# snudm-starlab/VMLMF

Hardware: AMD Instinct MI355X
Metric: RNN timesteps/sec (fwd+bwd) at B=64 T=128 hid=180 r=16; 1/2/4/8 GPU (higher is better)
Workload: dtype f32; 1 GPU; BASELINE configs[1]: UCI-HAR shape, Net(MyLSTM[MyVMLMFCell]) 1 layer, B=64/GPU T=128 I=9 H=180 w_rank=16 u_rank=16, CE loss, fwd+bwd; parameters packed inside every step, as a training loop sees it (with kept parameter images: ms_per_step_kept_images); global_batch=64, batch_per_gpu=64, seq_len=128, parallelism=dp1, scaling=weak, launch=hipgraph, parameter_images=packed inside every step (what a training loop sees), criterion=vmlmf_amd.Net.loss (cross-entropy riding on the forward launch, C ABI vmlmf_ce)

## Files before the change

### vmlmf_amd/csrc/vmlmf_launch.h

```cpp
#pragma once
#include <hip/hip_runtime.h>
#include "vmlmf_device.h"
#include "vmlmf_dropout.h"

#define VG_REC_BOUNDS (MAXT + 128)

enum EnvRule { ENV_SET, ENV_ON, ENV_INT, ENV_POS };
int vmlmf_env_switch(const char* name, EnvRule rule, int dflt);

struct HeadFwd {
  const float *W, *bias;
  float* logits;
  int C, pad;
};
struct HeadBwd {
  const float *W, *dl;
  const float* hlast;
  float *dW, *db;
  long long ldh;
  int C, pad;
};

struct FwdArgs {
  const float *gx, *VE, *UR, *EH, *h0, *c0;
// ... 11 lines not shown
  unsigned long long* ticket;
};
struct XwArgs {
  const float *x, *UXP, *WXD, *BBT;
  HeadFwd hd;
  CeFwd ce;
  const float *BH, *DX;
  int direct, pad;
};
struct AtbArgs {
  const float *dpre, *x, *y, *h0, *qx, *dqx, *Qs, *dQs;
  float* P;
  int pad0, pad;
};
constexpr int WR_PROG_STRIDE = 32;
constexpr unsigned VMLMF_ST_WRIDE = 1, VMLMF_ST_CLUSTER = 2, VMLMF_ST_WF_FWD = 3, VMLMF_ST_WF_BWD = 4, VMLMF_ST_P2P = 5;
__device__ __forceinline__ void vg_raise(unsigned* status, unsigned code) {
  if (status != nullptr) __hip_atomic_store(status, code, __ATOMIC_RELAXED, __HIP_MEMORY_SCOPE_SYSTEM);
}
struct WRide {
  AtbArgs a;
  float* dux;
  const float* vx;
  unsigned* prog;
  int K, S, ntg, tasks;
  int lag;
  int direct;
  unsigned spin;
  unsigned* status;
};
// ... 290 lines not shown
```

### vmlmf_amd/csrc/vmlmf_rec3.inc

```
#include "vmlmf_rec_fwd.inc"
#include "vmlmf_rec_bwd.inc"

constexpr int R3_MAXS = 3;


__device__ __forceinline__ float r3_total(float4 p) { return (p.x + p.y) + (p.z + p.w); }

__device__ __forceinline__ float fmac_ror_x16_4(float src, const float* w) {
  float a0 = 0.f, a1 = 0.f, a2 = 0.f, a3 = 0.f;
  asm("v_fmac_f32 %0, %4, %5\n\t" VG_DPP1(1, 4, 6, 1) VG_DPP1(2, 4, 7, 2) VG_DPP1(3, 4, 8, 3) VG_DPP1(0, 4, 9, 4) VG_DPP1(1, 4, 10, 5)
      VG_DPP1(2, 4, 11, 6) VG_DPP1(3, 4, 12, 7) VG_DPP1(0, 4, 13, 8) VG_DPP1(1, 4, 14, 9) VG_DPP1(2, 4, 15, 10) VG_DPP1(3, 4, 16, 11)
      VG_DPP1(0, 4, 17, 12) VG_DPP1(1, 4, 18, 13) VG_DPP1(2, 4, 19, 14) VG_DPP1(3, 4, 20, 15)
      : "+v"(a0), "+v"(a1), "+v"(a2), "+v"(a3)
      : "v"(src), "v"(w[0]), "v"(w[1]), "v"(w[2]), "v"(w[3]), "v"(w[4]), "v"(w[5]), "v"(w[6]), "v"(w[7]), "v"(w[8]), "v"(w[9]),
        "v"(w[10]), "v"(w[11]), "v"(w[12]), "v"(w[13]), "v"(w[14]), "v"(w[15]));
  return (a0 + a1) + (a2 + a3);
}

__host__ __device__ inline size_t rec3_fwd_lds_floats(int NT, int T, int IM) { return 128 + (size_t)12 * NT + (size_t)(T + 32) * IM + 8; }

template <int KH, int IM>
__global__ void __launch_bounds__(256) rec3_fwd_kernel(VGeo g, FwdArgs a, XwArgs xwargs) {
  static_assert(KH == 8 || KH == 16, "one 16-rank pass");
  static_assert(IM % 4 == 0 && IM >= 4 && IM <= 16, "narrow inputs");
// ... 225 lines not shown
  }
  hipLaunchKernelGGL(kern, dim3(g.nwg), dim3(g.NT + 64), lds, s, g, a, xw);
  return (int)hipGetLastError();
}
template <int KH>
static int rec3_fwd_launch_kh(const VGeo& g, const FwdArgs& a, const XwArgs& xw, hipStream_t s) {
  switch ((g.I + 3) / 4) {
    case 1: return rec3_fwd_launch_one<KH, 4>(g, a, xw, s);
    case 2: return rec3_fwd_launch_one<KH, 8>(g, a, xw, s);
    case 3: return rec3_fwd_launch_one<KH, 12>(g, a, xw, s);
    case 4: return rec3_fwd_launch_one<KH, 16>(g, a, xw, s);
  }
  return -3;
}

__host__ __device__ inline size_t rec3_bwd_lds_floats(int NT) {
  return 128 + (size_t)BWD_NB * NT * 6 + (size_t)2 * NT * 4 + 256 + 4 + (size_t)DR_SCR_FLOATS * NT;
}

#define VG_ADD1(acc, src, k) "v_add_f32_dpp %" #acc ", %" #src ", %" #acc " row_ror:" #k " row_mask:0xf bank_mask:0xf\n\t"
__device__ __forceinline__ float add_ror_x16(const float (&z)[16]) {
  float a0 = z[0], a1 = 0.f, a2 = 0.f;
  asm("s_nop 1\n\t" VG_ADD1(1, 3, 1) VG_ADD1(2, 4, 2) VG_ADD1(0, 5, 3) VG_ADD1(1, 6, 4) VG_ADD1(2, 7, 5) VG_ADD1(0, 8, 6) VG_ADD1(1, 9, 7)
      VG_ADD1(2, 10, 8) VG_ADD1(0, 11, 9) VG_ADD1(1, 12, 10) VG_ADD1(2, 13, 11) VG_ADD1(0, 14, 12) VG_ADD1(1, 15, 13) VG_ADD1(2, 16, 14)
      VG_ADD1(0, 17, 15)
      : "+v"(a0), "+v"(a1), "+v"(a2)
      : "v"(z[1]), "v"(z[2]), "v"(z[3]), "v"(z[4]), "v"(z[5]), "v"(z[6]), "v"(z[7]), "v"(z[8]), "v"(z[9]), "v"(z[10]), "v"(z[11]),
        "v"(z[12]), "v"(z[13]), "v"(z[14]), "v"(z[15]));
  return (a0 + a1) + a2;
}

template <int KH, int RIDE = 0>
__global__ void __launch_bounds__(320) rec3_bwd_kernel(VGeo g, BwdArgs a) {
  static_assert(KH == 8 || KH == 16, "one 16-rank pass");
  if constexpr (RIDE > 0) {
    if ((int)blockIdx.x >= g.nwg) {
      wride_worker<RIDE>(g, a.wr);
      return;
    }
  }
  const int tid = threadIdx.x, lane = tid & 63, wave = tid >> 6;
  const int NT = g.NT, NW = g.NW, H = g.H, B = g.B, T = g.T;
  const bool has_dy = a.dy != nullptr;
  const size_t sstride = (size_t)g.Bp * NT;
  const int row = blockIdx.x;

  extern __shared__ float4 smem4[];
  float* part = reinterpret_cast<float*>(smem4);
  float* tg = part + 128;
  float* tcp = tg + BWD_NB * NT * 4;
  float* tdy = tcp + BWD_NB * NT;
  float* outs = tdy + BWD_NB * NT;
  float* spare = outs + 2 * NT * 4;
  float* drscr = spare + 256 + 4;
  if (tid < 128) part[tid] = 0.f;

  if (tid >= NT) {
    constexpr int MAXS = R3_MAXS;
    constexpr int NDMA = 3 * MAXS;
    constexpr int DEPTH = 2;
    constexpr int DIST = DEPTH + 2;
    static_assert(DIST < BWD_NB && 2 * NDMA <= 63, "tape ring");
    if (wave == NW) {
      auto issue = [&](int ttarget) {
        const int tc = ttarget > 0 ? ttarget : 0;
        const int ring = ((ttarget % BWD_NB) + BWD_NB) % BWD_NB;
#pragma unroll
        for (int i = 0; i < MAXS; ++i) {
          const bool real = i < NW;
          const int slot = lane + 64 * (real ? i : 0);
          const size_t e = (size_t)tc * sstride + (size_t)row * NT + slot;
          int n;
          if (!vg_slot_unit(g, slot, n)) n = 0;
          const size_t lo = (size_t)ring * NT + 64 * (real ? i : 0);
          dma16(a.gates + e * 4, real ? tg + lo * 4 : spare);
          dma4(a.cs + e, real ? tcp + lo : spare);
          dma4(has_dy ? a.dy + ((size_t)tc * g.syT + (size_t)row * g.syB + n) : a.cs + e, real ? tdy + lo : spare);
        }
      };
      for (int s0 = 0; s0 < DIST; ++s0) issue(T - 1 - s0);
      wait_vm_barrier<(DIST - 2) * NDMA>();
      for (int t = T - 1; t >= 0; --t) {
        issue(t - DIST);
        wait_vm_barrier<DEPTH * NDMA>();
      }
      return;
    }
    const bool qv = lane < KH;
    const unsigned qdst = (unsigned)(row * KH + (lane < KH ? lane : 0)) * 4u;
    constexpr bool SAFE_ST = false;
    auto drain = [&](int ts) {
      const float* src = outs + (size_t)(ts & 1) * NT * 4;
      float* dt = a.dpre + (size_t)ts * sstride * 4;
      float4 d4[MAXS];
#pragma unroll
      for (int i = 0; i < MAXS; ++i) d4[i] = ld4(src + ((size_t)lane + 64 * (i < NW ? i : 0)) * 4);
      const float4 pq = ld4(part + (ts & 1) * 64 + (lane & 15) * 4);
#pragma unroll
      for (int i = 0; i < MAXS; ++i)
        if (i < NW) {
          if constexpr (RIDE > 0) st4_sv_sys<SAFE_ST>(dt, 16u * (unsigned)(row * NT + lane + 64 * i), d4[i]);
          else st4_sv(dt, 16u * (unsigned)(row * NT + lane + 64 * i), d4[i]);
        }
      float* qt = a.dQs + (size_t)ts * B * KH;
      if (qv) {
        if constexpr (RIDE > 0) st1_sv_sys<SAFE_ST>(qt, qdst, r3_total(pq));
        else st1_sv(qt, qdst, r3_total(pq));
      }
    };
    const int nd = NW + 1;
    const int lag = a.wr.lag;
    const int nwait = nd * lag;
    asm volatile("s_waitcnt lgkmcnt(0)\n\ts_barrier" ::: "memory");
    for (int t = T - 1; t >= 0; --t) {
      if (t + 1 < T) {
        drain(t + 1);
        if constexpr (RIDE > 0) {
          wait_vm_dyn(nwait);
          const int done = T - (t + 1 + lag);
          if (lane == 0 && (t & 1) == 0)
            st1_sv_sys<SAFE_ST>(a.wr.prog, 4u * (unsigned)(row * WR_PROG_STRIDE), (unsigned)(done > 0 ? done : 0));
        }
      }
      asm volatile("s_waitcnt lgkmcnt(0)\n\ts_barrier" ::: "memory");
    }
    drain(0);
    if constexpr (RIDE > 0) {
      asm volatile("s_waitcnt vmcnt(0)" ::: "memory");
      if (lane == 0) st1_sv_sys<SAFE_ST>(a.wr.prog, 4u * (unsigned)(row * WR_PROG_STRIDE), (unsigned)T);
    }
    return;
  }

  const bool valid = tid < H;
  const int n = valid ? tid : 0;

  float dh_head;
  if constexpr (RIDE > 0)
    dh_head = a.hd.C > 0 ? head_dh_body((const __attribute__((address_space(4))) char*)__builtin_amdgcn_kernarg_segment_ptr(), row, n, valid) : 0.f;
// ... 49 lines not shown
  for (int gk = 0; gk < 4; ++gk) eh[gk] = a.EH[gk * NT + tid];
  }

  float dhrec, dcs, ccur;
  {
    const size_t bh = (size_t)row * H + n;
    dhrec = (valid && a.dhT != nullptr) ? a.dhT[bh] : 0.f;
    dhrec += dh_head;
    dcs = (valid && a.dcT != nullptr) ? a.dcT[bh] : 0.f;
    ccur = a.cs[(size_t)T * sstride + (size_t)row * NT + tid];
  }
  asm volatile("s_waitcnt vmcnt(0) lgkmcnt(0)\n\ts_barrier" ::: "memory");

  float4 g4n;
  float cprvn, dyvn;
  auto fetch_tape = [&](int tt) {
    const int ringn = ((tt % BWD_NB) + BWD_NB) % BWD_NB;
    const size_t lo = (size_t)ringn * NT + tid;
    g4n = ld4(tg + lo * 4);
    cprvn = tcp[lo];
    dyvn = tdy[lo];
  };
  CellBwdFactors fac;
  float fdy;
  auto prepare = [&]() {
    fac = cell_bwd_factors(g4n, ccur, cprvn);
    fdy = (valid && has_dy) ? dyvn : 0.f;
    ccur = cprvn;
  };
  fetch_tape(T - 1);
  prepare();
  for (int t = T - 1; t >= 0; --t) {
    const int buf = t & 1;
    fetch_tape(t - 1);
    const float4 dp = cell_bwd_step(fac, fdy + dhrec, dcs);
    st4(outs + (size_t)buf * NT * 4 + (size_t)tid * 4, dp);
    const float ehterm = cell_ehterm_fma(dp, eh[0], eh[1], eh[2], eh[3]);
    f32x2 z2[8];
#pragma unroll
    for (int j = 0; j < 8; ++j) z2[j] = splat2(dp.x) * vz[0][j];
#pragma unroll
    for (int j = 0; j < 8; ++j) z2[j] = pk_fma(splat2(dp.y), vz[1][j], z2[j]);
#pragma unroll
    for (int j = 0; j < 8; ++j) z2[j] = pk_fma(splat2(dp.z), vz[2][j], z2[j]);
#pragma unroll
    for (int j = 0; j < 8; ++j) z2[j] = pk_fma(splat2(dp.w), vz[3][j], z2[j]);
    float z[16];
#pragma unroll
    for (int j = 0; j < 8; ++j) z[2 * j] = z2[j].x, z[2 * j + 1] = z2[j].y;
    const float s = rowsum4(add_ror_x16(z));
    if (lane < 16) part[buf * 64 + lane * 4 + wave] = s;
    prepare();
    asm volatile("s_waitcnt lgkmcnt(0)\n\ts_barrier" ::: "memory");
    const float4 p = ld4(part + buf * 64 + (lane & 15) * 4);
    float tot = r3_total(p);
    dpp_fence(tot);
    dhrec = ehterm + fmac_ror_x16_4(tot, ue);
  }

  if (valid) {
    if (a.dh0 != nullptr) a.dh0[(size_t)row * H + n] = dhrec;
    if (a.dc0 != nullptr) a.dc0[(size_t)row * H + n] = dcs;
  }
}

__host__ inline bool rec3_bwd_ok(const VGeo& g) {
  return !g.generic && !g.rb && !g.bf && g.G == 1 && !g.flat && g.KH <= 16 && g.R == 1 && g.NW <= R3_MAXS;
}

template <int KH>
static int rec3_bwd_launch_kh(const VGeo& g, const BwdArgs& a, hipStream_t s) {
  const size_t lds = sizeof(float) * rec3_bwd_lds_floats(g.NT);
  if (a.wr.K > 0) {
    const int n1 = (vg_nb1(g) + 31) / 32, n2 = (g.G * g.KH + 31) / 32;
    if (n1 > 2 || n2 > 2) return -3;
    const size_t lds1 = lds > 84 * 1024 ? lds : (size_t)84 * 1024;
    const dim3 grid(g.nwg + a.wr.K * a.wr.ntg), block(g.NT + 128);
    auto k1 = rec3_bwd_kernel<KH, 1>;
    auto k2 = rec3_bwd_kernel<KH, 2>;
    auto kern = (n1 == 1 && n2 == 1) ? k1 : k2;
    const hipError_t e = hipFuncSetAttribute(reinterpret_cast<const void*>(kern), hipFuncAttributeMaxDynamicSharedMemorySize, (int)lds1);
    if (e != hipSuccess) return (int)e;
    hipLaunchKernelGGL(kern, grid, block, lds1, s, g, a);
    return (int)hipGetLastError();
  }
  hipLaunchKernelGGL((rec3_bwd_kernel<KH>), dim3(g.nwg), dim3(g.NT + 128), lds, s, g, a);
  return (int)hipGetLastError();
// ... 2 lines not shown
```

### vmlmf_amd/csrc/vmlmf_rec_fwd.inc

```
#include "vmlmf_launch.h"
#include "vmlmf_direct.inc"

constexpr int FWD_NB = 6;


template <typename S>
__device__ __forceinline__ void copy_from_kernarg(S* dst, const __attribute__((address_space(4))) char* src) {
  static_assert(sizeof(S) % 4 == 0, "dword-sized argument structs");
  const __attribute__((address_space(4))) int* w = (const __attribute__((address_space(4))) int*)src;
  int tmp[sizeof(S) / 4];
#pragma unroll
  for (unsigned i = 0; i < sizeof(S) / 4; ++i) tmp[i] = w[i];
  __builtin_memcpy(dst, tmp, sizeof(S));
}
constexpr size_t karg_align8(size_t v) { return (v + 7) & ~(size_t)7; }
constexpr size_t KARG_FWD = karg_align8(sizeof(VGeo));
constexpr size_t KARG_XW = karg_align8(KARG_FWD + sizeof(FwdArgs));

__device__ __forceinline__ float wave_total(float v) {
  v = add_ror16<8>(v);
  v = add_ror16<4>(v);
  v = add_ror16<2>(v);
  v = add_ror16<1>(v);
  return rowsum4(v);
// ... 101 lines not shown
    ce.loss[0] = (float)(sum / (double)nv);
    ce.nvalid[0] = nv;
    __hip_atomic_store(ce.ticket, (u64)0, __ATOMIC_RELAXED, __HIP_MEMORY_SCOPE_AGENT);
    if (flag != 0) __hip_atomic_store(ce.ticket + 1, (u64)0, __ATOMIC_RELAXED, __HIP_MEMORY_SCOPE_AGENT);
  }
}

constexpr int XW_SLOTS = 3;
constexpr int XW_NB = 12;
constexpr int XW_DIST = 8;

__host__ __device__ inline size_t xwave_lds_floats() { return (size_t)XW_NB * 64 + 2 * 32; }

template <int IM, int IE = IM>
__device__ __attribute__((noinline)) void xwave_role(const __attribute__((address_space(4))) char* ka, float* gxs,
                                                     float* xlds, int row, int ring_nb) {
  VGeo g;
  XwArgs xa;
  copy_from_kernarg(&g, ka);
  copy_from_kernarg(&xa, ka + KARG_XW);
  const int lane = threadIdx.x & 63;
  const int I = g.I, H = g.H, NT = g.NT, T = g.T, KX = g.KX;
  typedef __attribute__((address_space(3))) float lds_f;
  typedef __attribute__((address_space(3))) f32x4 lds_f4;
  lds_f* xring = (lds_f*)xlds;
  lds_f* qxs = xring + XW_NB * 64;
  lds_f* gxl = (lds_f*)gxs;
  const bool rowok = row < g.B;
  const int rowc = rowok ? row : g.B - 1;

  f32x2 w01[XW_SLOTS][IM], w23[XW_SLOTS][IM], b01[XW_SLOTS], b23[XW_SLOTS];
// ... 52 lines not shown
    const lds_f4* xr4 = (const lds_f4*)(xring + (t % XW_NB) * 64);
#pragma unroll
    for (int m4 = 0; m4 < IM / 4; ++m4) {
      const f32x4 v = xr4[m4];
      sx[4 * m4 + 0] = (rowok && 4 * m4 + 0 < I) ? v[0] : 0.f;
      sx[4 * m4 + 1] = (rowok && 4 * m4 + 1 < I) ? v[1] : 0.f;
      sx[4 * m4 + 2] = (rowok && 4 * m4 + 2 < I) ? v[2] : 0.f;
      sx[4 * m4 + 3] = (rowok && 4 * m4 + 3 < I) ? v[3] : 0.f;
    }
    float q = 0.f;
    if (g.foldx == 0) {
#pragma unroll
      for (int m = 0; m < IM; ++m) q = fmaf(sx[m], uxc[m], q);
    }
    if (g.foldx == 0 && lane < KX) qxs[(t & 1) * 32 + lane] = q;
    lds_f* dst = gxl + (size_t)(t % ring_nb) * NT * 4;
#pragma unroll
    for (int i = 0; i < XW_SLOTS; ++i) {
      if (real[i]) {
        f32x2 p01a = b01[i], p01b = f32x2{0.f, 0.f}, p23a = b23[i], p23b = f32x2{0.f, 0.f};
#pragma unroll
        for (int m = 0; m + 1 < IE; m += 2) {
          p01a = pk_fma(splat2(sx[m]), w01[i][m], p01a);
          p23a = pk_fma(splat2(sx[m]), w23[i][m], p23a);
          p01b = pk_fma(splat2(sx[m + 1]), w01[i][m + 1], p01b);
          p23b = pk_fma(splat2(sx[m + 1]), w23[i][m + 1], p23b);
        }
        if constexpr ((IE & 1) != 0) {
          p01a = pk_fma(splat2(sx[IE - 1]), w01[i][IE - 1], p01a);
          p23a = pk_fma(splat2(sx[IE - 1]), w23[i][IE - 1], p23a);
        }
// ... 11 lines not shown
    produce(t + 1);
    wait_vm_barrier<XW_DIST - 2>();
  }
}

template <int KH, int R, bool FLAT, int MAXT, int CNT, bool XW = false>
__global__ void __launch_bounds__(VG_REC_BOUNDS) rec_fwd_kernel(VGeo g, FwdArgs a, XwArgs xwargs) {
  constexpr int NP = (KH + 15) / 16, KQ = NP * 16, NC = KH / 4;
  const int tid = threadIdx.x, lane = tid & 63, wave = tid >> 6;
  const int NT = g.NT, NW = g.NW, W = g.W, H = g.H, B = g.B, T = g.T;
  const bool mover = tid >= NT;
  const bool train = a.gates != nullptr;
  const size_t sstride = (size_t)g.Bp * NT;

  extern __shared__ float4 smem4[];
  float* part = reinterpret_cast<float*>(smem4);
  float* gxs = part + 2 * R * NW * KQ;
  float* outs = gxs + FWD_NB * R * NT * 4;
  float* zero4 = outs + 2 * R * NT * 8 + 256;
  if (tid < 4) zero4[tid] = 0.f;

  if (mover) {
    constexpr int MAXS = MAXT / 64;
    constexpr int NDMA = R * MAXS;
    constexpr int DEPTH = (2 * NDMA <= 63) ? 2 : 1;
    constexpr int DIST = DEPTH + 2;
    static_assert(DIST < FWD_NB, "gx ring too shallow");
    float* spare = outs + 2 * R * NT * 8;
    int row[R];
    bool rok[R];
#pragma unroll
    for (int r = 0; r < R; ++r) {
      row[r] = blockIdx.x * R + r;
      rok[r] = row[r] < B;
    }
    if (wave == NW) {
      if constexpr (XW) {
        const __attribute__((address_space(4))) char* ka =
            (const __attribute__((address_space(4))) char*)__builtin_amdgcn_kernarg_segment_ptr();
        float* xlds = zero4 + 4;
        switch ((g.I + 3) / 4) {
          case 1: xwave_role<4>(ka, gxs, xlds, row[0], FWD_NB); break;
          case 2: xwave_role<8>(ka, gxs, xlds, row[0], FWD_NB); break;
          case 3:
            if (g.I == 9) xwave_role<12, 9>(ka, gxs, xlds, row[0], FWD_NB);
            else if (g.I == 10) xwave_role<12, 10>(ka, gxs, xlds, row[0], FWD_NB);
            else xwave_role<12>(ka, gxs, xlds, row[0], FWD_NB);
            break;
          default: xwave_role<16>(ka, gxs, xlds, row[0], FWD_NB); break;
        }
        return;
      }
      auto issue = [&](int ttarget) {
        const int tc = ttarget < T ? ttarget : T - 1;
        float* dst = gxs + (size_t)(ttarget % FWD_NB) * R * NT * 4;
#pragma unroll
        for (int r = 0; r < R; ++r)
#pragma unroll
          for (int i = 0; i < MAXS; ++i) {
            const bool real = i < NW;
            const int i0 = real ? i : 0;
            dma16(a.gx + ((size_t)tc * sstride + (size_t)row[r] * NT + lane + 64 * i0) * 4,
                  real ? dst + ((size_t)r * NT + 64 * i0) * 4 : spare);
          }
      };
      for (int s0 = 0; s0 < DIST; ++s0) issue(s0);
      wait_vm_barrier<(DIST - 2) * NDMA>();
      for (int t = 0; t < T; ++t) {
        issue(t + DIST);
        wait_vm_barrier<DEPTH * NDMA>();
      }
      return;
    }
    __builtin_amdgcn_s_setprio(3);
    if (a.prog != nullptr && lane < R && rok[lane < R ? lane : 0])
      a.prog[(size_t)(blockIdx.x * R + lane) * WR_PROG_STRIDE] = 0u;
    bool sv[R][MAXS];
    unsigned so_[R][MAXS], yo_[R][MAXS];
// ... 9 lines not shown
        yo_[r][i] = (unsigned)((rok[r] ? row[r] : 0) * g.syB + n) * 4u;
      }
    constexpr int QE = 2;
    bool qv[QE];
    unsigned qsrc[QE], qdst[QE];
#pragma unroll
    for (int q = 0; q < QE; ++q) {
      const int e = lane + 64 * q;
      const int GK = g.G * KH;
      const bool in = e < R * GK;
      const int ec = in ? e : 0;
      const int r = ec / GK, jr = ec - r * GK, j = jr / KH, rr = jr - j * KH;
      const int s = (g.G == 2 && rr >= g.off1) ? 1 : 0;
      const int w0 = ((j + s) % g.G) * W;
      qv[q] = in && train && (blockIdx.x * R + r) < B;
      qsrc[q] = (unsigned)((r * NW + w0) * KQ + rr);
      qdst[q] = (unsigned)((blockIdx.x * R + r) * GK + jr);
    }
    const float* qxs = zero4 + 4 + XW_NB * 64;
    const bool qx_out = XW && train && g.foldx == 0 && rok[0] && lane < g.KX;
    constexpr bool SAFE_ST = FLAT && MAXT == 512;
    auto segment = [&](int td, int tq) {
      __builtin_amdgcn_s_setprio(3);
      const int tdc = td < 0 ? 0 : td, tqc = tq < 0 ? 0 : tq;
      const float* src = outs + (size_t)(tdc & 1) * R * NT * 8;
      const float* qsrc_ = part + (size_t)(tqc & 1) * R * NW * KQ;
      float4 g4[R][MAXS];
      float2 ch[R][MAXS];
      float v[QE][MAXS];
      float qxv = 0.f;
#pragma unroll
      for (int r = 0; r < R; ++r)
#pragma unroll
        for (int i = 0; i < MAXS; ++i) {
          const int slot = lane + 64 * (i < NW ? i : 0);
          g4[r][i] = ld4(src + ((size_t)r * NT + slot) * 4);
          ch[r][i] = *reinterpret_cast<const float2*>(src + (size_t)R * NT * 4 + ((size_t)r * NT + slot) * 2);
        }
#pragma unroll
      for (int q = 0; q < QE; ++q)
#pragma unroll
        for (int w = 0; w < MAXS; ++w) v[q][w] = qsrc_[qsrc[q] + (w < W ? w : 0) * KQ];
      if constexpr (XW) qxv = qxs[(tqc & 1) * 32 + (lane & 31)];
      __builtin_amdgcn_s_setprio(0);
      if (td >= 0) {
        char* gt = reinterpret_cast<char*>(a.gates + (size_t)td * sstride * 4);
        char* ct = reinterpret_cast<char*>(a.cs + (size_t)(td + 1) * sstride);
        char* yt = reinterpret_cast<char*>(a.y + (size_t)td * g.syT);
#pragma unroll
        for (int r = 0; r < R; ++r) {
#pragma unroll
          for (int i = 0; i < MAXS; ++i) {
            if (i < NW) {
              if (train) {
                st4_sv<SAFE_ST, !SAFE_ST>(gt, 4u * so_[r][i], g4[r][i]);
                st1_sv<SAFE_ST, !SAFE_ST>(ct, so_[r][i], ch[r][i].x);
              }
// ... 102 lines not shown
  }

  constexpr int NCP = NC <= 2 ? 2 : (NC <= 4 ? 4 : 8);
  constexpr bool FASTQ16 = !FLAT && NC == NCP && NC * CNT <= 16;
  constexpr bool FASTQ64 = !FLAT && !FASTQ16 && NC <= 8 && NCP * CNT <= 64;
  constexpr bool FLATQ = FLAT && NC <= 8 && NCP * CNT <= 32;
  constexpr bool FASTQ = FASTQ16 || FASTQ64 || FLATQ;
  int rdoff = 0;
  {
    const int li = FLATQ ? (lane & 31) : (FASTQ64 ? lane : (lane & 15)), cc = li % NCP, w = li / NCP;
    const int ccl = cc < NC ? cc : 0;
    const int s = (g.G == 2 && 4 * ccl >= g.off1) ? 1 : 0;
    const int q0 = FLATQ ? (lane >> 5) : grp;
    rdoff = (w < CNT && cc < NC) ? ((((q0 + s) % g.G) * W + w) * KQ + 4 * cc) : -1;
  }

  float h[R], c[R];
#pragma unroll
  for (int r = 0; r < R; ++r) {
    const int row = blockIdx.x * R + r;
    const bool ok = valid && row < B;
    const int rowc = row < B ? row : B - 1;
    h[r] = (ok && a.h0 != nullptr) ? a.h0[(size_t)rowc * H + n] : 0.f;
    c[r] = (ok && a.c0 != nullptr) ? a.c0[(size_t)rowc * H + n] : 0.f;
    if (train) a.cs[(size_t)row * NT + tid] = c[r];
  }

  for (int t = 0; t < T; ++t) {
    const int buf = t & 1;
#pragma unroll
    for (int r = 0; r < R; ++r) {
      float hv = h[r];
      dpp_fence(hv);
#pragma unroll
      for (int p = 0; p < NP; ++p) {
        float a0 = 0.f, a1 = 0.f;
        fmac_ror_x16(a0, a1, hv, &ur[p * 16]);
        const float s = rowsum4(a0 + a1);
        if (lane < 16) part[((buf * R + r) * NW + wave) * KQ + p * 16 + lane] = s;
      }
    }
    asm volatile("s_waitcnt lgkmcnt(0)\n\ts_barrier" ::: "memory");
    const float* gxt = gxs + (size_t)(t % FWD_NB) * R * NT * 4;
    float* ot = outs + (size_t)buf * R * NT * 8;
#pragma unroll
    for (int r = 0; r < R; ++r) {
      const float* src = part + (size_t)(buf * R + r) * NW * KQ;
      const float4 gx4 = ld4(gxt + ((size_t)r * NT + tid) * 4);
      float4 q[NC], q2[FLAT ? NC : 1];
      if constexpr (FASTQ) {
        const float4 v = ld4(rdoff >= 0 ? src + rdoff : zero4);
        float sx = class_sum16<NCP>(v.x), sy = class_sum16<NCP>(v.y);
        float sz = class_sum16<NCP>(v.z), sw = class_sum16<NCP>(v.w);
        if constexpr (FASTQ64) sx = rowsum4(sx), sy = rowsum4(sy), sz = rowsum4(sz), sw = rowsum4(sw);
        if constexpr (FLATQ) sx = rowsum2(sx), sy = rowsum2(sy), sz = rowsum2(sz), sw = rowsum2(sw);
#pragma unroll
        for (int cc = 0; cc < NC; ++cc)
          q[cc] = make_float4(bcast_lane(sx, cc), bcast_lane(sy, cc), bcast_lane(sz, cc), bcast_lane(sw, cc));
        if constexpr (FLATQ) {
#pragma unroll
          for (int cc = 0; cc < NC; ++cc)
            q2[cc] = make_float4(bcast_lane(sx, 32 + cc), bcast_lane(sy, 32 + cc), bcast_lane(sz, 32 + cc), bcast_lane(sw, 32 + cc));
        }
      }
#pragma unroll
// ... 19 lines not shown
      for (int cc = 0; cc < NC; ++cc) {
        const float4 qa = q[cc];
        const float4 qb = FLAT ? q2[cc] : q[cc];
        p01a = pk_fma(splat2(qa.x), ve01[4 * cc + 0], p01a);
        p23a = pk_fma(splat2(qb.x), ve23[4 * cc + 0], p23a);
        p01b = pk_fma(splat2(qa.y), ve01[4 * cc + 1], p01b);
        p23b = pk_fma(splat2(qb.y), ve23[4 * cc + 1], p23b);
        p01a = pk_fma(splat2(qa.z), ve01[4 * cc + 2], p01a);
        p23a = pk_fma(splat2(qb.z), ve23[4 * cc + 2], p23a);
        p01b = pk_fma(splat2(qa.w), ve01[4 * cc + 3], p01b);
        p23b = pk_fma(splat2(qb.w), ve23[4 * cc + 3], p23b);
      }
      const f32x2 pre01 = p01a + p01b, pre23 = p23a + p23b;
      const CellFwd cell = cell_fwd(pre01.x, pre01.y, pre23.x, pre23.y, c[r]);
      c[r] = cell.c, h[r] = cell.h;
      st4(ot + ((size_t)r * NT + tid) * 4, cell.gates);
      *reinterpret_cast<float2*>(ot + (size_t)R * NT * 4 + ((size_t)r * NT + tid) * 2) = make_float2(c[r], h[r]);
    }
  }
  asm volatile("s_waitcnt lgkmcnt(0)\n\ts_barrier" ::: "memory");

#pragma unroll
  for (int r = 0; r < R; ++r) {
    const int row = blockIdx.x * R + r;
    if (valid && row < B) {
      if (a.hT != nullptr) a.hT[(size_t)row * H + n] = h[r];
      if (a.cT != nullptr) a.cT[(size_t)row * H + n] = c[r];
    }
  }
  if constexpr (R == 1) {
    {
      typedef __attribute__((address_space(3))) float lds_f;
      const float* chp = outs + (size_t)((T - 1) & 1) * R * NT * 8 + (size_t)R * NT * 4;
      head_epilogue((const __attribute__((address_space(4))) char*)__builtin_amdgcn_kernarg_segment_ptr(), (const lds_f*)chp,
                    (int)blockIdx.x, wave, (lds_f*)part);
      ce_epilogue((const __attribute__((address_space(4))) char*)__builtin_amdgcn_kernarg_segment_ptr(), (int)blockIdx.x, wave, (lds_f*)part);
    }
  }
}

template <int KH, int R, bool FLAT, int MAXT, int CNT>
static int fwd_launch_one(const VGeo& g, const FwdArgs& a, const XwArgs& xw, hipStream_t s) {
  constexpr int KQ = (KH + 15) / 16 * 16;
  if (a.xwave != 0) {
    if constexpr (R == 1 && MAXT == 256 && !FLAT) {
      const size_t ldsx = sizeof(float) * ((size_t)2 * g.NW * KQ + (size_t)FWD_NB * g.NT * 4 + (size_t)2 * g.NT * 8 + 256 + 4 +
                                           xwave_lds_floats() + ((a.xwave & 2) != 0 ? (size_t)(4 * g.I + 4) * g.NT : 0));
      hipLaunchKernelGGL((rec_fwd_kernel<KH, R, FLAT, MAXT, CNT, true>), dim3(g.nwg), dim3(g.NT + 128), ldsx, s, g, a, xw);
      return (int)hipGetLastError();
    } else {
      return -3;
    }
  }
  const size_t lds = sizeof(float) * ((size_t)2 * R * g.NW * KQ + (size_t)FWD_NB * R * g.NT * 4 + (size_t)2 * R * g.NT * 8 + 256 + 4);
  auto kern = rec_fwd_kernel<KH, R, FLAT, MAXT, CNT>;
  if (lds > 64 * 1024) {
    const hipError_t e = hipFuncSetAttribute(reinterpret_cast<const void*>(kern),
                                             hipFuncAttributeMaxDynamicSharedMemorySize, (int)lds);
    if (e != hipSuccess) return (int)e;
  }
  hipLaunchKernelGGL(kern, dim3(g.nwg), dim3(g.NT + 128), lds, s, g, a, xw);
  return (int)hipGetLastError();
}

template <int KH, int MAXT, int CNT, bool ALSO_FLAT>
static int fwd_launch_mode(const VGeo& g, const FwdArgs& a, const XwArgs& xw, hipStream_t s) {
  if (g.R != 1) return -3;
  if (g.flat) {
    if constexpr (ALSO_FLAT) return g.G == 2 ? fwd_launch_one<KH, 1, true, MAXT, CNT>(g, a, xw, s) : -3;
// ... 31 lines not shown
```

### vmlmf_amd/csrc/vmlmf_state.hip

```cpp
#include <atomic>
#include <cstdlib>

#include "vmlmf_host.h"

using namespace vmlmf_host;

int vmlmf_env_switch(const char* name, EnvRule rule, int dflt) {
  const char* e = getenv(name);
  if (e == nullptr) return dflt;
  switch (rule) {
    case ENV_SET: return 1;
    case ENV_ON: return e[0] != '0';
    case ENV_INT: return atoi(e);
    case ENV_POS: break;
  }
  const int v = atoi(e);
  return v >= 1 ? v : dflt;
}

namespace vmlmf_host {

static thread_local std::string g_err = "";

int fail(int code, const std::string& msg) {
// ... 10 lines not shown
  const char* key;
  int dflt;
  EnvRule rule;
  int* var;
};
const Switch g_switches[] = {
    {"VMLMF_DEBUG_SYNC", nullptr, 0, ENV_SET, &g_debug_sync},
    {"VMLMF_ADAM_GUARD", "adam_guard", 1, ENV_INT, &g_adam_guard},
    {"VMLMF_XWAVE", nullptr, 1, ENV_ON, &g_xwave},
    {"VMLMF_WCHUNKS", nullptr, 64, ENV_POS, &g_wchunks},
    {"VMLMF_WMIN", nullptr, 64, ENV_POS, &g_wmin},
    {"VMLMF_RC", nullptr, 0, ENV_POS, &g_rc},
    {"VMLMF_WRIDE", nullptr, 1, ENV_ON, &g_wride},
    {"VMLMF_WRIDE_K", nullptr, 32, ENV_POS, &g_wride_k},
    {"VMLMF_WRIDE_MAXB", nullptr, 64, ENV_POS, &g_wride_maxb},
    {"VMLMF_WRIDE_LAG", nullptr, 3, ENV_POS, &g_wride_lag},
    {"VMLMF_WRIDE_RC", nullptr, 32, ENV_POS, &g_wride_rc},
    {"VMLMF_RB", "rb", -1, ENV_INT, &g_rb_mode},
    {"VMLMF_RB_MINB", "rb_min_batch", 0, ENV_POS, &g_rb_minB},
    {"VMLMF_RB_S", "rb_cluster", 0, ENV_POS, &g_rb_S},
    {"VMLMF_RB_ROWS", "rb_rows", 0, ENV_POS, &g_rb_rows},
    {"VMLMF_REC3", "rec3", 6, ENV_INT, &g_rec3},
    {"VMLMF_INROW", "inrow", -1, ENV_INT, &g_inrow},
    {"VMLMF_WRING", "wring", -1, ENV_INT, &g_wring},
    {"VMLMF_DIRECT", "direct", 1, ENV_INT, &g_direct},
    {"VMLMF_FINISH2", "finish2", 1, ENV_INT, &g_finish2},
    {"VMLMF_WF_BWD", nullptr, 1, ENV_INT, &g_wf_bwd},
    {"VMLMF_PACK_SLIM", nullptr, 1, ENV_INT, &g_pack_slim},
    {"VMLMF_FINISH_UNITS", nullptr, 1, ENV_INT, &g_finish_units},
    {"VMLMF_RBX", "rbx", 1, ENV_INT, &g_rbx},
    {"VMLMF_FFB", "ffb", 0, ENV_INT, &g_ffb},
// ... 196 lines not shown
```

Before: 916,600 RNN timesteps/s.

## Use power-of-two fixed-stride LDS rings, unroll periods, rank-major forward partials

The forward x-wave path and the riding backward path now use an 8-deep LDS tape/gx ring with a fixed 192-slot stride, so ring indices become masks. The step loops are unrolled by the ring period so ring offsets fold into constants. The forward rank-1 case gains a rank-major partial-sum layout that replaces the 16-lane butterfly with one vector load and broadcasts. The backward drain wait gets a compile-time vmcnt for the default lag, and the DPP add chain drops its zero initialisations. The intent is to cut per-step integer, LDS and reduction overhead on the serial recurrence, at the cost of larger LDS use and more code.

```diff
diff --git a/vmlmf_amd/csrc/vmlmf_launch.h b/vmlmf_amd/csrc/vmlmf_launch.h
--- a/vmlmf_amd/csrc/vmlmf_launch.h
+++ b/vmlmf_amd/csrc/vmlmf_launch.h
@@ -49,6 +49,7 @@
   int pad0, pad;
 };
 constexpr int WR_PROG_STRIDE = 32;
+constexpr int WR_LAG_DEFAULT = 3;
 constexpr unsigned VMLMF_ST_WRIDE = 1, VMLMF_ST_CLUSTER = 2, VMLMF_ST_WF_FWD = 3, VMLMF_ST_WF_BWD = 4, VMLMF_ST_P2P = 5;
 __device__ __forceinline__ void vg_raise(unsigned* status, unsigned code) {
   if (status != nullptr) __hip_atomic_store(status, code, __ATOMIC_RELAXED, __HIP_MEMORY_SCOPE_SYSTEM);
diff --git a/vmlmf_amd/csrc/vmlmf_rec3.inc b/vmlmf_amd/csrc/vmlmf_rec3.inc
--- a/vmlmf_amd/csrc/vmlmf_rec3.inc
+++ b/vmlmf_amd/csrc/vmlmf_rec3.inc
@@ -4,7 +4,11 @@
 constexpr int R3_MAXS = 3;
 
 
-__device__ __forceinline__ float r3_total(float4 p) { return (p.x + p.y) + (p.z + p.w); }
+__device__ __forceinline__ float r3_total(float4 p) {
+  float lo = p.x + p.y;
+  asm("" : "+v"(lo));
+  return lo + (p.z + p.w);
+}
 
 __device__ __forceinline__ float fmac_ror_x16_4(float src, const float* w) {
   float a0 = 0.f, a1 = 0.f, a2 = 0.f, a3 = 0.f;
@@ -263,19 +267,24 @@
   return -3;
 }
 
-__host__ __device__ inline size_t rec3_bwd_lds_floats(int NT) {
-  return 128 + (size_t)BWD_NB * NT * 6 + (size_t)2 * NT * 4 + 256 + 4 + (size_t)DR_SCR_FLOATS * NT;
+constexpr int R3_NB = 8;
+constexpr int R3_NTS = 64 * R3_MAXS;
+__host__ __device__ inline size_t rec3_bwd_lds_floats(int NT, bool fixed = false) {
+  const size_t nts = fixed ? R3_NTS : NT;
+  return 128 + (size_t)R3_NB * nts * 6 + (size_t)2 * nts * 4 + 256 + 4 + (size_t)DR_SCR_FLOATS * NT;
 }
 
 #define VG_ADD1(acc, src, k) "v_add_f32_dpp %" #acc ", %" #src ", %" #acc " row_ror:" #k " row_mask:0xf bank_mask:0xf\n\t"
+#define VG_ADD0(acc, src, k) "v_add_f32_dpp %" #acc ", %" #src ", %18 row_ror:" #k " row_mask:0xf bank_mask:0xf\n\t"
 __device__ __forceinline__ float add_ror_x16(const float (&z)[16]) {
-  float a0 = z[0], a1 = 0.f, a2 = 0.f;
-  asm("s_nop 1\n\t" VG_ADD1(1, 3, 1) VG_ADD1(2, 4, 2) VG_ADD1(0, 5, 3) VG_ADD1(1, 6, 4) VG_ADD1(2, 7, 5) VG_ADD1(0, 8, 6) VG_ADD1(1, 9, 7)
+  float a0 = z[0], a1, a2;
+  const float zero = 0.f;
+  asm("s_nop 1\n\t" VG_ADD0(1, 3, 1) VG_ADD0(2, 4, 2) VG_ADD1(0, 5, 3) VG_ADD1(1, 6, 4) VG_ADD1(2, 7, 5) VG_ADD1(0, 8, 6) VG_ADD1(1, 9, 7)
       VG_ADD1(2, 10, 8) VG_ADD1(0, 11, 9) VG_ADD1(1, 12, 10) VG_ADD1(2, 13, 11) VG_ADD1(0, 14, 12) VG_ADD1(1, 15, 13) VG_ADD1(2, 16, 14)
       VG_ADD1(0, 17, 15)
-      : "+v"(a0), "+v"(a1), "+v"(a2)
+      : "+v"(a0), "=&v"(a1), "=&v"(a2)
       : "v"(z[1]), "v"(z[2]), "v"(z[3]), "v"(z[4]), "v"(z[5]), "v"(z[6]), "v"(z[7]), "v"(z[8]), "v"(z[9]), "v"(z[10]), "v"(z[11]),
-        "v"(z[12]), "v"(z[13]), "v"(z[14]), "v"(z[15]));
+        "v"(z[12]), "v"(z[13]), "v"(z[14]), "v"(z[15]), "v"(zero));
   return (a0 + a1) + a2;
 }
 
@@ -294,13 +303,14 @@
   const size_t sstride = (size_t)g.Bp * NT;
   const int row = blockIdx.x;
 
+  const int NTS = RIDE > 0 ? R3_NTS : NT;
   extern __shared__ float4 smem4[];
   float* part = reinterpret_cast<float*>(smem4);
   float* tg = part + 128;
-  float* tcp = tg + BWD_NB * NT * 4;
-  float* tdy = tcp + BWD_NB * NT;
-  float* outs = tdy + BWD_NB * NT;
-  float* spare = outs + 2 * NT * 4;
+  float* tcp = tg + R3_NB * NTS * 4;
+  float* tdy = tcp + R3_NB * NTS;
+  float* outs = tdy + R3_NB * NTS;
+  float* spare = outs + 2 * NTS * 4;
   float* drscr = spare + 256 + 4;
   if (tid < 128) part[tid] = 0.f;
 
@@ -309,11 +319,11 @@
     constexpr int NDMA = 3 * MAXS;
     constexpr int DEPTH = 2;
     constexpr int DIST = DEPTH + 2;
-    static_assert(DIST < BWD_NB && 2 * NDMA <= 63, "tape ring");
+    static_assert(DIST < R3_NB && (R3_NB & (R3_NB - 1)) == 0 && 2 * NDMA <= 63, "tape ring");
     if (wave == NW) {
       auto issue = [&](int ttarget) {
         const int tc = ttarget > 0 ? ttarget : 0;
-        const int ring = ((ttarget % BWD_NB) + BWD_NB) % BWD_NB;
+        const int ring = ttarget & (R3_NB - 1);
 #pragma unroll
         for (int i = 0; i < MAXS; ++i) {
           const bool real = i < NW;
@@ -321,7 +331,7 @@
           const size_t e = (size_t)tc * sstride + (size_t)row * NT + slot;
           int n;
           if (!vg_slot_unit(g, slot, n)) n = 0;
-          const size_t lo = (size_t)ring * NT + 64 * (real ? i : 0);
+          const size_t lo = (size_t)ring * NTS + 64 * (real ? i : 0);
           dma16(a.gates + e * 4, real ? tg + lo * 4 : spare);
           dma4(a.cs + e, real ? tcp + lo : spare);
           dma4(has_dy ? a.dy + ((size_t)tc * g.syT + (size_t)row * g.syB + n) : a.cs + e, real ? tdy + lo : spare);
@@ -339,7 +349,7 @@
     const unsigned qdst = (unsigned)(row * KH + (lane < KH ? lane : 0)) * 4u;
     constexpr bool SAFE_ST = false;
     auto drain = [&](int ts) {
-      const float* src = outs + (size_t)(ts & 1) * NT * 4;
+      const float* src = outs + (size_t)(ts & 1) * NTS * 4;
       float* dt = a.dpre + (size_t)ts * sstride * 4;
       float4 d4[MAXS];
 #pragma unroll
@@ -360,18 +370,30 @@
     const int nd = NW + 1;
     const int lag = a.wr.lag;
     const int nwait = nd * lag;
+    auto segments = [&](auto nwait_c) {
+      constexpr int NWAIT = decltype(nwait_c)::value;
+      for (int t = T - 1; t >= 0; --t) {
+        if (t + 1 < T) {
+          drain(t + 1);
+          if constexpr (RIDE > 0) {
+            if constexpr (NWAIT >= 0) asm volatile("s_waitcnt vmcnt(%0)" ::"n"(NWAIT) : "memory");
+            else wait_vm_dyn(nwait);
+            const int done = T - (t + 1 + lag);
+            if (lane == 0 && (t & 1) == 0)
+              st1_sv_sys<SAFE_ST>(a.wr.prog, 4u * (unsigned)(row * WR_PROG_STRIDE), (unsigned)(done > 0 ? done : 0));
+          }
+        }
+        asm volatile("s_waitcnt lgkmcnt(0)\n\ts_barrier" ::: "memory");
+      }
+    };
     asm volatile("s_waitcnt lgkmcnt(0)\n\ts_barrier" ::: "memory");
-    for (int t = T - 1; t >= 0; --t) {
-      if (t + 1 < T) {
-        drain(t + 1);
-        if constexpr (RIDE > 0) {
-          wait_vm_dyn(nwait);
-          const int done = T - (t + 1 + lag);
-          if (lane == 0 && (t & 1) == 0)
-            st1_sv_sys<SAFE_ST>(a.wr.prog, 4u * (unsigned)(row * WR_PROG_STRIDE), (unsigned)(done > 0 ? done : 0));
-        }
-      }
-      asm volatile("s_waitcnt lgkmcnt(0)\n\ts_barrier" ::: "memory");
+    if constexpr (RIDE == 1 && KH == 16) {
+      switch (nwait) {
+        case 4 * WR_LAG_DEFAULT: segments(std::integral_constant<int, 4 * WR_LAG_DEFAULT>{}); break;
+        default: segments(std::integral_constant<int, -1>{}); break;
+      }
+    } else {
+      segments(std::integral_constant<int, -1>{});
     }
     drain(0);
     if constexpr (RIDE > 0) {
@@ -451,9 +473,8 @@
 
   float4 g4n;
   float cprvn, dyvn;
-  auto fetch_tape = [&](int tt) {
-    const int ringn = ((tt % BWD_NB) + BWD_NB) % BWD_NB;
-    const size_t lo = (size_t)ringn * NT + tid;
+  auto fetch_tape = [&](const int ringn) __attribute__((always_inline)) {
+    const size_t lo = (size_t)ringn * NTS + tid;
     g4n = ld4(tg + lo * 4);
     cprvn = tcp[lo];
     dyvn = tdy[lo];
@@ -465,13 +486,12 @@
     fdy = (valid && has_dy) ? dyvn : 0.f;
     ccur = cprvn;
   };
-  fetch_tape(T - 1);
+  fetch_tape((T - 1) & (R3_NB - 1));
   prepare();
-  for (int t = T - 1; t >= 0; --t) {
-    const int buf = t & 1;
-    fetch_tape(t - 1);
+  auto step = [&](const int ringp, const int buf) __attribute__((always_inline)) {
+    fetch_tape(ringp);
     const float4 dp = cell_bwd_step(fac, fdy + dhrec, dcs);
-    st4(outs + (size_t)buf * NT * 4 + (size_t)tid * 4, dp);
+    st4(outs + (size_t)buf * NTS * 4 + (size_t)tid * 4, dp);
     const float ehterm = cell_ehterm_fma(dp, eh[0], eh[1], eh[2], eh[3]);
     f32x2 z2[8];
 #pragma unroll
@@ -493,6 +513,22 @@
     float tot = r3_total(p);
     dpp_fence(tot);
     dhrec = ehterm + fmac_ror_x16_4(tot, ue);
+  };
+  constexpr bool PERIODS = RIDE == 1 && KH == 16;
+  int t = T - 1;
+  for (; PERIODS ? (t & (R3_NB - 1)) != R3_NB - 1 : t >= 0; --t) step((t - 1) & (R3_NB - 1), t & 1);
+  if constexpr (PERIODS) {
+    for (; t >= 0; t -= R3_NB) {
+      step(6, 1);
+      step(5, 0);
+      step(4, 1);
+      step(3, 0);
+      step(2, 1);
+      step(1, 0);
+      step(0, 1);
+      step(7, 0);
+    }
+    static_assert(R3_NB == 8, "the unrolled period above");
   }
 
   if (valid) {
@@ -507,7 +543,7 @@
 
 template <int KH>
 static int rec3_bwd_launch_kh(const VGeo& g, const BwdArgs& a, hipStream_t s) {
-  const size_t lds = sizeof(float) * rec3_bwd_lds_floats(g.NT);
+  const size_t lds = sizeof(float) * rec3_bwd_lds_floats(g.NT, a.wr.K > 0);
   if (a.wr.K > 0) {
     const int n1 = (vg_nb1(g) + 31) / 32, n2 = (g.G * g.KH + 31) / 32;
     if (n1 > 2 || n2 > 2) return -3;
diff --git a/vmlmf_amd/csrc/vmlmf_rec_fwd.inc b/vmlmf_amd/csrc/vmlmf_rec_fwd.inc
--- a/vmlmf_amd/csrc/vmlmf_rec_fwd.inc
+++ b/vmlmf_amd/csrc/vmlmf_rec_fwd.inc
@@ -2,6 +2,15 @@
 #include "vmlmf_direct.inc"
 
 constexpr int FWD_NB = 6;
+constexpr int FWD_XNB = 8;
+constexpr int FWD_XNTS = 192;
+
+template <int KH, int R, bool FLAT, int MAXT, int CNT>
+constexpr bool fwd_rank_major() { return !FLAT && R == 1 && MAXT == 256 && (KH == 8 || KH == 16) && CNT <= 4; }
+template <int KH, int R, bool FLAT, int MAXT, int CNT>
+__host__ __device__ constexpr size_t fwd_part_floats(int NW) {
+  return fwd_rank_major<KH, R, FLAT, MAXT, CNT>() ? (size_t)128 : (size_t)2 * R * NW * ((KH + 15) / 16 * 16);
+}
 
 
 template <typename S>
@@ -139,7 +148,7 @@
 
 template <int IM, int IE = IM>
 __device__ __attribute__((noinline)) void xwave_role(const __attribute__((address_space(4))) char* ka, float* gxs,
-                                                     float* xlds, int row, int ring_nb) {
+                                                     float* xlds, int row) {
   VGeo g;
   XwArgs xa;
   copy_from_kernarg(&g, ka);
@@ -222,7 +231,7 @@
       for (int m = 0; m < IM; ++m) q = fmaf(sx[m], uxc[m], q);
     }
     if (g.foldx == 0 && lane < KX) qxs[(t & 1) * 32 + lane] = q;
-    lds_f* dst = gxl + (size_t)(t % ring_nb) * NT * 4;
+    lds_f* dst = gxl + (size_t)(t & (FWD_XNB - 1)) * FWD_XNTS * 4;
 #pragma unroll
     for (int i = 0; i < XW_SLOTS; ++i) {
       if (real[i]) {
@@ -264,10 +273,14 @@
   const size_t sstride = (size_t)g.Bp * NT;
 
   extern __shared__ float4 smem4[];
+  constexpr bool RM = fwd_rank_major<KH, R, FLAT, MAXT, CNT>();
   float* part = reinterpret_cast<float*>(smem4);
-  float* gxs = part + 2 * R * NW * KQ;
-  float* outs = gxs + FWD_NB * R * NT * 4;
-  float* zero4 = outs + 2 * R * NT * 8 + 256;
+  static_assert(!XW || (R == 1 && MAXT == 256 && !FLAT), "the x-projection wave's instantiations");
+  constexpr int NB = XW ? FWD_XNB : FWD_NB;
+  const int NTS = XW ? FWD_XNTS : NT;
+  float* gxs = part + fwd_part_floats<KH, R, FLAT, MAXT, CNT>(NW);
+  float* outs = gxs + NB * R * NTS * 4;
+  float* zero4 = outs + 2 * R * NTS * 8 + 256;
   if (tid < 4) zero4[tid] = 0.f;
 
   if (mover) {
@@ -275,8 +288,8 @@
     constexpr int NDMA = R * MAXS;
     constexpr int DEPTH = (2 * NDMA <= 63) ? 2 : 1;
     constexpr int DIST = DEPTH + 2;
-    static_assert(DIST < FWD_NB, "gx ring too shallow");
-    float* spare = outs + 2 * R * NT * 8;
+    static_assert(DIST < NB && (!XW || (NB & (NB - 1)) == 0), "gx ring too shallow");
+    float* spare = outs + 2 * R * NTS * 8;
     int row[R];
     bool rok[R];
 #pragma unroll
@@ -290,20 +303,20 @@
             (const __attribute__((address_space(4))) char*)__builtin_amdgcn_kernarg_segment_ptr();
         float* xlds = zero4 + 4;
         switch ((g.I + 3) / 4) {
-          case 1: xwave_role<4>(ka, gxs, xlds, row[0], FWD_NB); break;
-          case 2: xwave_role<8>(ka, gxs, xlds, row[0], FWD_NB); break;
+          case 1: xwave_role<4>(ka, gxs, xlds, row[0]); break;
+          case 2: xwave_role<8>(ka, gxs, xlds, row[0]); break;
           case 3:
-            if (g.I == 9) xwave_role<12, 9>(ka, gxs, xlds, row[0], FWD_NB);
-            else if (g.I == 10) xwave_role<12, 10>(ka, gxs, xlds, row[0], FWD_NB);
-            else xwave_role<12>(ka, gxs, xlds, row[0], FWD_NB);
+            if (g.I == 9) xwave_role<12, 9>(ka, gxs, xlds, row[0]);
+            else if (g.I == 10) xwave_role<12, 10>(ka, gxs, xlds, row[0]);
+            else xwave_role<12>(ka, gxs, xlds, row[0]);
             break;
-          default: xwave_role<16>(ka, gxs, xlds, row[0], FWD_NB); break;
+          default: xwave_role<16>(ka, gxs, xlds, row[0]); break;
         }
         return;
       }
       auto issue = [&](int ttarget) {
         const int tc = ttarget < T ? ttarget : T - 1;
-        float* dst = gxs + (size_t)(ttarget % FWD_NB) * R * NT * 4;
+        float* dst = gxs + (size_t)(ttarget % NB) * R * NTS * 4;
 #pragma unroll
         for (int r = 0; r < R; ++r)
 #pragma unroll
@@ -311,7 +324,7 @@
             const bool real = i < NW;
             const int i0 = real ? i : 0;
             dma16(a.gx + ((size_t)tc * sstride + (size_t)row[r] * NT + lane + 64 * i0) * 4,
-                  real ? dst + ((size_t)r * NT + 64 * i0) * 4 : spare);
+                  real ? dst + ((size_t)r * NTS + 64 * i0) * 4 : spare);
           }
       };
       for (int s0 = 0; s0 < DIST; ++s0) issue(s0);
@@ -351,7 +364,7 @@
       const int s = (g.G == 2 && rr >= g.off1) ? 1 : 0;
       const int w0 = ((j + s) % g.G) * W;
       qv[q] = in && train && (blockIdx.x * R + r) < B;
-      qsrc[q] = (unsigned)((r * NW + w0) * KQ + rr);
+      qsrc[q] = RM ? (unsigned)(rr * 4 + w0) : (unsigned)((r * NW + w0) * KQ + rr);
       qdst[q] = (unsigned)((blockIdx.x * R + r) * GK + jr);
     }
     const float* qxs = zero4 + 4 + XW_NB * 64;
@@ -360,8 +373,8 @@
     auto segment = [&](int td, int tq) {
       __builtin_amdgcn_s_setprio(3);
       const int tdc = td < 0 ? 0 : td, tqc = tq < 0 ? 0 : tq;
-      const float* src = outs + (size_t)(tdc & 1) * R * NT * 8;
-      const float* qsrc_ = part + (size_t)(tqc & 1) * R * NW * KQ;
+      const float* src = outs + (size_t)(tdc & 1) * R * NTS * 8;
+      const float* qsrc_ = part + (RM ? (size_t)(tqc & 1) * 64 : (size_t)(tqc & 1) * R * NW * KQ);
       float4 g4[R][MAXS];
       float2 ch[R][MAXS];
       float v[QE][MAXS];
@@ -371,13 +384,13 @@
 #pragma unroll
         for (int i = 0; i < MAXS; ++i) {
           const int slot = lane + 64 * (i < NW ? i : 0);
-          g4[r][i] = ld4(src + ((size_t)r * NT + slot) * 4);
-          ch[r][i] = *reinterpret_cast<const float2*>(src + (size_t)R * NT * 4 + ((size_t)r * NT + slot) * 2);
+          g4[r][i] = ld4(src + ((size_t)r * NTS + slot) * 4);
+          ch[r][i] = *reinterpret_cast<const float2*>(src + (size_t)R * NTS * 4 + ((size_t)r * NTS + slot) * 2);
         }
 #pragma unroll
       for (int q = 0; q < QE; ++q)
 #pragma unroll
-        for (int w = 0; w < MAXS; ++w) v[q][w] = qsrc_[qsrc[q] + (w < W ? w : 0) * KQ];
+        for (int w = 0; w < MAXS; ++w) v[q][w] = qsrc_[qsrc[q] + (w < W ? w : 0) * (RM ? 1 : KQ)];
       if constexpr (XW) qxv = qxs[(tqc & 1) * 32 + (lane & 31)];
       __builtin_amdgcn_s_setprio(0);
       if (td >= 0) {
@@ -510,6 +523,15 @@
     const int q0 = FLATQ ? (lane >> 5) : grp;
     rdoff = (w < CNT && cc < NC) ? ((((q0 + s) % g.G) * W + w) * KQ + 4 * cc) : -1;
   }
+  static_assert(!RM || FASTQ16, "rank-major partials replace the 16-lane butterfly");
+  bool rmsel = false;
+  if constexpr (RM) {
+    const int li = lane & 15;
+    const int s = (g.G == 2 && 4 * (li >> 2) >= g.off1) ? 1 : 0;
+    rmsel = ((grp + s) % g.G) != 0;
+    if (wave == 0 && lane < 16)
+      for (int w = NW; w < 4; ++w) part[lane * 4 + w] = 0.f, part[64 + lane * 4 + w] = 0.f;
+  }
 
   float h[R], c[R];
 #pragma unroll
@@ -522,8 +544,7 @@
     if (train) a.cs[(size_t)row * NT + tid] = c[r];
   }
 
-  for (int t = 0; t < T; ++t) {
-    const int buf = t & 1;
+  auto step = [&](const int ring, const int buf) __attribute__((always_inline)) {
 #pragma unroll
     for (int r = 0; r < R; ++r) {
       float hv = h[r];
@@ -533,18 +554,35 @@
         float a0 = 0.f, a1 = 0.f;
         fmac_ror_x16(a0, a1, hv, &ur[p * 16]);
         const float s = rowsum4(a0 + a1);
-        if (lane < 16) part[((buf * R + r) * NW + wave) * KQ + p * 16 + lane] = s;
+        if constexpr (RM) {
+          if (lane < 16) part[buf * 64 + lane * 4 + wave] = s;
+        } else {
+          if (lane < 16) part[((buf * R + r) * NW + wave) * KQ + p * 16 + lane] = s;
+        }
       }
     }
     asm volatile("s_waitcnt lgkmcnt(0)\n\ts_barrier" ::: "memory");
-    const float* gxt = gxs + (size_t)(t % FWD_NB) * R * NT * 4;
-    float* ot = outs + (size_t)buf * R * NT * 8;
+    const float* gxt = gxs + (size_t)ring * R * NTS * 4;
+    float* ot = outs + (size_t)buf * R * NTS * 8;
 #pragma unroll
     for (int r = 0; r < R; ++r) {
       const float* src = part + (size_t)(buf * R + r) * NW * KQ;
-      const float4 gx4 = ld4(gxt + ((size_t)r * NT + tid) * 4);
+      const float4 gx4 = ld4(gxt + ((size_t)r * NTS + tid) * 4);
       float4 q[NC], q2[FLAT ? NC : 1];
-      if constexpr (FASTQ) {
+      if constexpr (RM) {
+        const float4 v = ld4(part + buf * 64 + (lane & 15) * 4);
+        float tot;
+        if constexpr (CNT >= 3) {
+          tot = (v.x + v.z) + (v.y + v.w);
+        } else {
+          const float a0 = CNT == 1 ? (rmsel ? v.y : v.x) : (rmsel ? v.z : v.x);
+          const float a1 = CNT == 1 ? 0.f : (rmsel ? v.w : v.y);
+          tot = (a0 + 0.f) + (a1 + 0.f);
+        }
+#pragma unroll
+        for (int cc = 0; cc < NC; ++cc)
+          q[cc] = make_float4(bcast_lane(tot, 4 * cc), bcast_lane(tot, 4 * cc + 1), bcast_lane(tot, 4 * cc + 2), bcast_lane(tot, 4 * cc + 3));
+      } else if constexpr (FASTQ) {
         const float4 v = ld4(rdoff >= 0 ? src + rdoff : zero4);
         float sx = class_sum16<NCP>(v.x), sy = class_sum16<NCP>(v.y);
         float sz = class_sum16<NCP>(v.z), sw = class_sum16<NCP>(v.w);
@@ -594,10 +632,25 @@
       const f32x2 pre01 = p01a + p01b, pre23 = p23a + p23b;
       const CellFwd cell = cell_fwd(pre01.x, pre01.y, pre23.x, pre23.y, c[r]);
       c[r] = cell.c, h[r] = cell.h;
-      st4(ot + ((size_t)r * NT + tid) * 4, cell.gates);
-      *reinterpret_cast<float2*>(ot + (size_t)R * NT * 4 + ((size_t)r * NT + tid) * 2) = make_float2(c[r], h[r]);
-    }
-  }
+      st4(ot + ((size_t)r * NTS + tid) * 4, cell.gates);
+      *reinterpret_cast<float2*>(ot + (size_t)R * NTS * 4 + ((size_t)r * NTS + tid) * 2) = make_float2(c[r], h[r]);
+    }
+  };
+  int t = 0;
+  if constexpr (XW && KH == 16 && CNT == 3) {
+    static_assert(FWD_XNB == 8, "the unrolled period below");
+    for (; t + FWD_XNB <= T; t += FWD_XNB) {
+      step(0, 0);
+      step(1, 1);
+      step(2, 0);
+      step(3, 1);
+      step(4, 0);
+      step(5, 1);
+      step(6, 0);
+      step(7, 1);
+    }
+  }
+  for (; t < T; ++t) step(XW ? (t & (FWD_XNB - 1)) : t % FWD_NB, t & 1);
   asm volatile("s_waitcnt lgkmcnt(0)\n\ts_barrier" ::: "memory");
 
 #pragma unroll
@@ -611,7 +664,7 @@
   if constexpr (R == 1) {
     {
       typedef __attribute__((address_space(3))) float lds_f;
-      const float* chp = outs + (size_t)((T - 1) & 1) * R * NT * 8 + (size_t)R * NT * 4;
+      const float* chp = outs + (size_t)((T - 1) & 1) * R * NTS * 8 + (size_t)R * NTS * 4;
       head_epilogue((const __attribute__((address_space(4))) char*)__builtin_amdgcn_kernarg_segment_ptr(), (const lds_f*)chp,
                     (int)blockIdx.x, wave, (lds_f*)part);
       ce_epilogue((const __attribute__((address_space(4))) char*)__builtin_amdgcn_kernarg_segment_ptr(), (int)blockIdx.x, wave, (lds_f*)part);
@@ -621,18 +674,23 @@
 
 template <int KH, int R, bool FLAT, int MAXT, int CNT>
 static int fwd_launch_one(const VGeo& g, const FwdArgs& a, const XwArgs& xw, hipStream_t s) {
-  constexpr int KQ = (KH + 15) / 16 * 16;
   if (a.xwave != 0) {
     if constexpr (R == 1 && MAXT == 256 && !FLAT) {
-      const size_t ldsx = sizeof(float) * ((size_t)2 * g.NW * KQ + (size_t)FWD_NB * g.NT * 4 + (size_t)2 * g.NT * 8 + 256 + 4 +
-                                           xwave_lds_floats() + ((a.xwave & 2) != 0 ? (size_t)(4 * g.I + 4) * g.NT : 0));
-      hipLaunchKernelGGL((rec_fwd_kernel<KH, R, FLAT, MAXT, CNT, true>), dim3(g.nwg), dim3(g.NT + 128), ldsx, s, g, a, xw);
+      const size_t ldsx = sizeof(float) * (fwd_part_floats<KH, R, FLAT, MAXT, CNT>(g.NW) + (size_t)FWD_XNB * FWD_XNTS * 4 + (size_t)2 * FWD_XNTS * 8 +
+                                           256 + 4 + xwave_lds_floats() + ((a.xwave & 2) != 0 ? (size_t)(4 * g.I + 4) * g.NT : 0));
+      auto kernx = rec_fwd_kernel<KH, R, FLAT, MAXT, CNT, true>;
+      if (g.NT > FWD_XNTS) return -3;
+      if (ldsx > 64 * 1024) {
+        const hipError_t e = hipFuncSetAttribute(reinterpret_cast<const void*>(kernx), hipFuncAttributeMaxDynamicSharedMemorySize, (int)ldsx);
+        if (e != hipSuccess) return (int)e;
+      }
+      hipLaunchKernelGGL(kernx, dim3(g.nwg), dim3(g.NT + 128), ldsx, s, g, a, xw);
       return (int)hipGetLastError();
     } else {
       return -3;
     }
   }
-  const size_t lds = sizeof(float) * ((size_t)2 * R * g.NW * KQ + (size_t)FWD_NB * R * g.NT * 4 + (size_t)2 * R * g.NT * 8 + 256 + 4);
+  const size_t lds = sizeof(float) * (fwd_part_floats<KH, R, FLAT, MAXT, CNT>(g.NW) + (size_t)FWD_NB * R * g.NT * 4 + (size_t)2 * R * g.NT * 8 + 256 + 4);
   auto kern = rec_fwd_kernel<KH, R, FLAT, MAXT, CNT>;
   if (lds > 64 * 1024) {
     const hipError_t e = hipFuncSetAttribute(reinterpret_cast<const void*>(kern),
diff --git a/vmlmf_amd/csrc/vmlmf_state.hip b/vmlmf_amd/csrc/vmlmf_state.hip
--- a/vmlmf_amd/csrc/vmlmf_state.hip
+++ b/vmlmf_amd/csrc/vmlmf_state.hip
@@ -48,7 +48,7 @@
     {"VMLMF_WRIDE", nullptr, 1, ENV_ON, &g_wride},
     {"VMLMF_WRIDE_K", nullptr, 32, ENV_POS, &g_wride_k},
     {"VMLMF_WRIDE_MAXB", nullptr, 64, ENV_POS, &g_wride_maxb},
-    {"VMLMF_WRIDE_LAG", nullptr, 3, ENV_POS, &g_wride_lag},
+    {"VMLMF_WRIDE_LAG", nullptr, WR_LAG_DEFAULT, ENV_POS, &g_wride_lag},
     {"VMLMF_WRIDE_RC", nullptr, 32, ENV_POS, &g_wride_rc},
     {"VMLMF_RB", "rb", -1, ENV_INT, &g_rb_mode},
     {"VMLMF_RB_MINB", "rb_min_batch", 0, ENV_POS, &g_rb_minB},
```

New measurement: 951,700 RNN timesteps/s, median of 6. +3.8%, better.
